# facebookresearch/iSDF

Hardware: AMD Instinct MI355X
Metric: train-steps/sec: device-synchronised Trainer.step() on 27k-point ray batches, timed as metrics.start_timing / end_timing bracket it (SURVEY 8d); whole job.  SDF L1 vs GT: sdf_l1_vs_gt (higher is better)
Workload: dtype f16 MFMA operands (compensated forward: hi+lo operands past the cat layer), f32 accumulate; second-order sweeps and dW operands fp16; 1 GPU; replicaCAD.json defaults: 5 keyframes x 200 rays x 27 samples = 27000 points per rank-step, 680x1200 synthetic room depth, 6x256 Softplus MLP + 255-wide icosahedron PE (460033 params), eik+normal loss, bounds=ray, AdamW; stream=680x1200, scaling_mode=weak: every rank draws the full 5 x 200 rays, parallelism=single GPU

## Files before the change

### isdf_amd/csrc/capi.hip

```cpp
#include <cstdio>
#include "isdf_common.h"
#include "chain_params.h"
#include "launchers.h"

using namespace isdf;

namespace isdf { thread_local int g_isdf_last_hip_error = 0; }

extern "C" {

int isdf_abi_version(void) { return ISDF_ABI_VERSION; }

static thread_local int g_isdf_last_collective_error = 0;

const char* isdf_error_string(int code) {
  switch (code) {
    case ISDF_OK: return "ok";
    case ISDF_EINVAL: return "invalid argument";
    case ISDF_EUNSUPPORTED: return "unsupported configuration (the tile kernels take hidden_feature_size <= 512 (zero-padded to 256 / 512), n_freqs = n_embed_funcs+1 in 1..12, any hidden_layers_block up to 7; bounds_method ray|pc)";
    case ISDF_EWORKSPACE: return "workspace too small";
    case ISDF_EHIP: {
      static thread_local char buf[160];
      snprintf(buf, sizeof(buf), "HIP runtime error: %s", g_isdf_last_hip_error ? hipGetErrorString((hipError_t)g_isdf_last_hip_error) : "(no launch status recorded)");
      return buf;
// ... 70 lines not shown
  if (!scan_ws || scan_ws_bytes < sample_scan_bytes((int64_t)a->n_frames * a->n_rays)) return ISDF_EWORKSPACE;
  return launch_sample_rays(*a, *o, scan_ws, (hipStream_t)stream);
}

int isdf_sdf_eval(const isdf_net_cfg* net, const float* params, const void* shadow, const float* pts,
                  int64_t n_points, const float* noise, float* sdf, float* sdf_grad, void* workspace,
                  int64_t workspace_bytes, void* stream) {
  isdf_clear_stale_hip_error();
  NetLayout l; int rc = make_layout(net, &l);
  if (rc) return rc;
  if (!layout_supported(l)) return ISDF_EUNSUPPORTED;
  if (!params || !shadow || !pts || !sdf || n_points < 0) return ISDF_EINVAL;
  if (n_points == 0) return ISDF_OK;
  ChainParams p = {};
  p.lay = l; p.params = params; p.shadow = (const uint16_t*)shadow; p.pts = pts; p.noise = noise;
  p.n_points_host = n_points; p.S = 1; p.sdf = sdf; p.sdf_grad = sdf_grad;
  const int mode = sdf_grad ? 1 : 0;
  WorkspaceLayout w; make_workspace(l, n_points, 0, false, &w);
  if (mode == 1) {
    if (!workspace || workspace_bytes < w.totalBytes) return ISDF_EWORKSPACE;
    p.spill = (uint16_t*)((char*)workspace + w.offSpill); p.sp = w.sp;
  }
  chain_debug_from_env(p.dbg, workspace && workspace_bytes >= 4096 ? (char*)workspace + workspace_bytes - 4096 : nullptr);
  return launch_chain(p, mode, w.nTiles, (hipStream_t)stream);
}

static bool optim_args_ok(const isdf_optim_args* opt, int32_t n_frames) {
  if (!opt || !opt->params || !opt->exp_avg || !opt->exp_avg_sq || !opt->shadow || opt->step < 1) return false;
  if ((opt->loss_approx == nullptr) != (opt->frame_avg == nullptr)) return false;
  if (opt->frame_avg_inline_n != 0 && (opt->frame_avg_inline_n != n_frames || opt->frame_avg_inline_n > ISDF_MAX_INLINE_FRAMES))
    return false;
// ... 32 lines not shown
  const int64_t maxPts = (int64_t)a->max_rays * a->S;
  if (maxPts > 0x7fffffff) return ISDF_EINVAL;
  if (a->extra_floats < 0 || a->extra_floats > 1016 || (a->extra_floats > 0 && (a->extra_slot < 0 || a->extra_slot >= a->extra_floats)))
    return ISDF_EINVAL;
  WorkspaceLayout w; make_workspace(l, maxPts, a->max_rays, true, &w);
  if (workspace_bytes < w.totalBytes) return ISDF_EWORKSPACE;
  hipStream_t st = (hipStream_t)stream;
  char* ws = (char*)workspace;
  float* wgLoss = (float*)(ws + w.offWgLoss);
  float* dwPart = (float*)(ws + w.offDwPart);
  float* vecPart = (float*)(ws + w.offVecPart);
  float* totLoss = (float*)(ws + w.offTotLoss);

  ChainParams p = {};
  p.lay = l; p.loss = *loss; p.params = params; p.shadow = (const uint16_t*)shadow;
  p.pts = a->pc; p.noise = a->noise; p.n_valid = a->n_valid; p.S = a->S;
  p.noise_std = a->noise_std; p.noise_seed = a->noise_seed; p.noise_off = a->noise_offset;
  p.z_vals = a->z_vals; p.depth = a->depth_sample; p.dirsC = a->dirs_C_sample; p.dirsW = a->dirs_W_sample;
  p.normals = a->norm_sample; p.pc_bounds = a->pc_bounds; p.pc_grad_vec = a->pc_grad_vec;
  p.sdf = o->sdf; p.sdf_grad = o->sdf_grad; p.tot_loss_mat = o->tot_loss_mat;
  p.tot_ws = totLoss; p.wg_loss = wgLoss; p.vec_part = vecPart; p.vecStride = w.vecStride;
  p.spill = (uint16_t*)(ws + w.offSpill); p.sp = w.sp;
  p.pe_aux = (float*)(ws + w.offPeAux);
  chain_debug_from_env(p.dbg, ws + w.totalBytes - 4096);
  hipEvent_t* ev = (hipEvent_t*)o->prof_events;
  if (ev && hipEventRecord(ev[0], st) != hipSuccess) return ISDF_EHIP;
  rc = launch_chain(p, 2, w.nTiles, st);
  if (rc) return rc;
  if (ev && hipEventRecord(ev[1], st) != hipSuccess) return ISDF_EHIP;

  DwParams d = {};
  d.lay = l; d.sp = w.sp; d.spill = p.spill; d.pe_aux = p.pe_aux; d.n_valid = a->n_valid; d.S = a->S; d.dwPart = dwPart;
  rc = launch_dw(d, st);
  if (rc) return rc;
  if (ev && hipEventRecord(ev[2], st) != hipSuccess) return ISDF_EHIP;
  const ReduceLayout r = reduce_layout(l, a->n_frames);
  TailParams t = {};
  t.lay = l; t.dwPart = dwPart; t.vecPart = vecPart; t.vecStride = w.vecStride; t.grad = o->reduce_buf;
  FinalizeArgs& f = t.fin;
  f.wg_loss = wgLoss; f.maxTiles = w.nTiles; f.n_valid = a->n_valid; f.S = a->S; f.tot_ws = totLoss;
  f.ib = a->indices_b; f.ih = a->indices_h; f.iw = a->indices_w; f.n_frames = a->n_frames; f.H = a->H; f.W = a->W;
  f.loss_sums = o->reduce_buf + r.lossSums; f.block_loss = o->reduce_buf + r.blockLoss; f.block_cnt = o->reduce_buf + r.blockCnt;
  f.mailbox = o->host_mailbox; f.extra = o->reduce_buf + r.extra;
  f.n_extra = a->extra_floats; f.extra_slot = a->extra_slot; f.extra_value = a->extra_value;
  if (opt) {
    const AdamwHyper hyper = tail_optim(t, *opt);
    rc = launch_step_tail(0, t, &hyper, 0, st);
// ... 301 lines not shown
```

### isdf_amd/csrc/chain.hip

```cpp
#include <atomic>
#include "chain_dev.h"
#include "launchers.h"

namespace isdf {

constexpr bool oper_f16(int oper) { return oper >= 1; }
constexpr bool oper_x2(int oper) { return oper >= 2; }
constexpr bool oper_x2_all(int oper) { return oper == 3; }

template <int HD, int EP, bool LO_REGIONS = false>
struct Tile {
  static constexpr int BM = TILE_PTS;
  static constexpr int NW = CHAIN_NW;
  static constexpr int CKF = CHAIN_CHUNK_FRAGS;
  static constexpr int FB = HD / (NW * 32);
  static constexpr int PB = BM / 32;
  static constexpr int R2 = (EP > HD ? EP : HD);
  static constexpr int XK = (HD + R2) * (LO_REGIONS ? 2 : 1);
  static constexpr int ROWB = XK * 2;
  static constexpr int XBYTES = BM * ROWB;
  static constexpr int OFF_XS = XBYTES;
  static constexpr bool WIDE_E = EP > HD;
  static constexpr int NPART = WIDE_E ? (NW * 64) / 32 : (NW * 64) / BM;
  static constexpr int OFF_PART = OFF_XS + BM * 16;
// ... 4 lines not shown
};

template <int FBN, int CKF> struct WChunk { uint4 v[CKF / FBN][FBN]; };
struct WRef { int soff; int rb; };

template <int FBN, int CKF>
__device__ __forceinline__ void load_w(WChunk<FBN, CKF>& wq, rsrc_t rw, WRef r, int lane16, int chunk) {
  constexpr int CK = CKF / FBN;
#pragma unroll
  for (int s = 0; s < CK; ++s)
#pragma unroll
    for (int fb = 0; fb < FBN; ++fb)
      wq.v[s][fb] = bload16<0>(rw, lane16 + (s & 3) * 1024, r.soff + fb * r.rb + chunk * CK * 1024 + (s >> 2) * 4096);
}

template <bool F16, int KSTEPS, int FBN, int PBN, int ROWB, int CKF, bool ZERO = false, bool TWO = false, typename Hook>
__device__ __forceinline__ void gemm(f32x16 (&acc)[FBN][PBN], WChunk<FBN, CKF>& wq, rsrc_t rw, WRef wr, const char* xl,
                                     int colByteBase, int lane, Hook&& postHook, int colByteBase2 = 0) {
  constexpr int CK = CKF / FBN;
  static_assert(KSTEPS % CK == 0, "K must be a multiple of the chunk");
  static_assert((ROWB & 255) == 0, "row base must leave the swizzle bits (4-7) clear");
  constexpr int NCH = KSTEPS / CK;
  typedef typename Op<F16>::v8 v8;
  const int j = lane & 31, hi = lane >> 5;
  const int xlane = j * ROWB + ((hi * 16) ^ ((j & 15) << 4));
  const int lane16 = lane * 16;
  load_w(wq, rw, wr, lane16, 0);
  auto chunk = [&](int ch, auto refill, auto zero) {
    const int k0 = ch * CK;
    int xch = (xlane ^ ((k0 & 7) * 32)) + (k0 >> 3) * 256 + colByteBase;
    asm volatile("" : "+v"(xch));
    constexpr int NB = TWO ? 2 * PBN : PBN;
    auto readb = [&](int s, v8 (&b)[NB]) {
#pragma unroll
      for (int pb = 0; pb < PBN; ++pb)
        b[pb] = __builtin_bit_cast(v8, *(const uint4*)(xl + ((xch ^ (s * 32)) + pb * 32 * ROWB)));
      if constexpr (TWO) {
#pragma unroll
        for (int pb = 0; pb < PBN; ++pb)
          b[PBN + pb] = __builtin_bit_cast(v8, *(const uint4*)(xl + ((xch ^ (s * 32)) + pb * 32 * ROWB + (colByteBase2 - colByteBase))));
      }
    };
// ... 57 lines not shown
  float* gbs = (float*)(smem + T::OFF_GB);
  float* red = (float*)(smem + T::OFF_RED);

  const NetLayout& L = p.lay;
  const int tid = threadIdx.x;
  const int w = __builtin_amdgcn_readfirstlane(tid >> 6);
  static_assert(FB <= 2, "the LDS write addressing below assumes one or two feature blocks per wave");
  int lane, j, hi, lane16, xw;
  auto refresh = [&] {
    int t = tid;
    asm volatile("" : "+v"(t));
    lane = t & 63; j = lane & 31; hi = lane >> 5; lane16 = lane * 16;
    xw = j * ROWB + 8 * hi + (((j & 15) << 4) ^ (((w * FB) & 3) * 64)) + ((w * FB) >> 2) * 256;
  };
  refresh();
  const int64_t P = p.n_valid ? (int64_t)(*p.n_valid) * p.S : p.n_points_host;
  const int64_t n0 = (int64_t)blockIdx.x * BM;
  if (n0 >= P) return;
  const int nf = L.n_freqs;
  const float so = L.scale_output;
  ChainStamps TS(p.dbg, p.n_cu);
  TS();
  if (SP8) __builtin_amdgcn_s_setreg(1 | (23 << 6), 1);
  const bool genOdd = ((int)blockIdx.x / p.n_cu) & 1;
  auto PRIO = [&](int phase) {
    if (genOdd) { if (phase == 1 || phase == 2) __builtin_amdgcn_s_setprio(1); else __builtin_amdgcn_s_setprio(0); }
  };
  PRIO(0);
  TS.wall(0);

  const int64_t setFwdA = L.setFwdA, setFwdB = L.setFwdB, setBwdA = L.setBwdA, setBwdB = L.setBwdB, setFwdLo = L.setFwdLo;
  uint16_t* spillTile = p.spill + TS.spill_tile() * p.sp.tileStride;
  const rsrc_t rsW = make_rsrc(p.shadow, 0x7fffffffu);
  const rsrc_t rsS = make_rsrc(spillTile, (uint32_t)(p.sp.tileStride * 2));
  const i32x4 srdS = make_srd(spillTile, (uint32_t)(p.sp.tileStride * 2));
  auto sbase = [&](int64_t tensorOff) { return (int)(tensorOff * 2) + w * (FB * PB * 2) * 1024; };
  constexpr auto cidx = [](int fb, int pb, int qp) { return (fb * PB + pb) * 2 + qp; };
  float* vecTile = MODE == 2 ? p.vec_part + (int64_t)blockIdx.x * p.vecStride : nullptr;
  const rsrc_t rsV = make_rsrc(vecTile, MODE == 2 ? (uint32_t)p.vecStride * 4u : 0u);
  (void)setFwdB; (void)setBwdB; (void)setFwdLo; (void)rsS; (void)rsV; (void)srdS;
  auto ubase = [&](int fb, int qp) { return w * (FB * 32) + fb * 32 + 16 * qp; };
  auto ld_params8 = [&](int vecBase, int ub, float (&o)[8]) {
    const rsrc_t rv = make_rsrc(p.params + vecBase, (uint32_t)L.H * 4u);
    const u32x4 a = __builtin_amdgcn_raw_buffer_load_b128(rv, 16 * hi, ub * 4, 0);
    const u32x4 b = __builtin_amdgcn_raw_buffer_load_b128(rv, 16 * hi + 32, ub * 4, 0);
#pragma unroll
    for (int e = 0; e < 4; ++e) { o[e] = __uint_as_float(a[e]); o[4 + e] = __uint_as_float(b[e]); }
  };
  auto vec_store8 = [&](float (&v)[8], int elemUniform) {
#pragma unroll
    for (int e = 0; e < 8; ++e) v[e] = half_wave_sum(v[e]);
    const bool b0 = j & 1, b1 = j & 2, b2 = j & 4;
    const float t0 = b0 ? v[1] : v[0], t1 = b0 ? v[3] : v[2], t2 = b0 ? v[5] : v[4], t3 = b0 ? v[7] : v[6];
    const float u0 = b1 ? t1 : t0, u1 = b1 ? t3 : t2;
    const float r = b2 ? u1 : u0;
    if (j < 8) __builtin_amdgcn_raw_buffer_store_b32(__float_as_uint(r), rsV, 16 * hi + 4 * (j & 3) + 32 * (j >> 2), elemUniform * 4, 0);
  };

  if constexpr (!WIDE_E && BM == 64) {
    const int ln = tid & 63;
    const int64_t n = n0 + ln;
    float x0 = 0.f, x1 = 0.f, x2 = 0.f;
    if (n < P) { x0 = p.pts[n * 3]; x1 = p.pts[n * 3 + 1]; x2 = p.pts[n * 3 + 2]; }
    const float y0 = (L.T[0] * x0 + L.T[1] * x1 + L.T[2] * x2 + L.T[3]) * L.scale_input;
    const float y1 = (L.T[4] * x0 + L.T[5] * x1 + L.T[6] * x2 + L.T[7]) * L.scale_input;
    const float y2 = (L.T[8] * x0 + L.T[9] * x1 + L.T[10] * x2 + L.T[11]) * L.scale_input;
    typedef typename Op<F16>::e opT;
    const int sw = (ln & 15) << 4;
    char* row = X + ln * ROWB;
    auto put = [&](int feat, float v) {
      *(opT*)(row + (((HD + feat) * 2) ^ sw)) = (opT)v;
      if (X2ALL) *(opT*)(row + (((LO + HD + feat) * 2) ^ sw)) = (opT)(v - (float)(opT)v);
    };
    if (w == T::NW - 1) {
      xs[ln * 4] = y0; xs[ln * 4 + 1] = y1; xs[ln * 4 + 2] = y2;
      put(0, y0); put(1, y1); put(2, y2);
      for (int f = L.E; f < EP; ++f) put(f, 0.f);
    }
    for (int d = w; d < N_DIRS; d += T::NW) {
      const float proj = y0 * kDirs[0][d] + y1 * kDirs[1][d] + y2 * kDirs[2][d];
      float fr = 1.f;
      for (int f = 0; f < nf; ++f) {
        const float xb = proj * fr;
        put(3 + d * nf + f, __sinf(xb));
        put(3 + N_DIRS * nf + d * nf + f, __sinf(xb + kHalfPi));
        fr *= 2.f;
      }
    }
  } else
  {
    const int pt = (tid % (BM / T::NW)) + (BM / T::NW) * (tid / 64), prt = (tid % 64) / (BM / T::NW);
    constexpr int NPART = (T::NW * 64) / BM;
    const int64_t n = n0 + pt;
    float x0 = 0.f, x1 = 0.f, x2 = 0.f;
    if (n < P) { x0 = p.pts[n * 3]; x1 = p.pts[n * 3 + 1]; x2 = p.pts[n * 3 + 2]; }
    float y0 = (L.T[0] * x0 + L.T[1] * x1 + L.T[2] * x2 + L.T[3]) * L.scale_input;
    float y1 = (L.T[4] * x0 + L.T[5] * x1 + L.T[6] * x2 + L.T[7]) * L.scale_input;
    float y2 = (L.T[8] * x0 + L.T[9] * x1 + L.T[10] * x2 + L.T[11]) * L.scale_input;
    typedef typename Op<F16>::e opT;
    char* row = X + pt * ROWB;
    auto put = [&](int feat, float v) {
      *(opT*)(row + swz(pt, (HD + feat) * 2)) = (opT)v;
      if (X2ALL) *(opT*)(row + swz(pt, (LO + HD + feat) * 2)) = (opT)(v - (float)(opT)v);
    };
    if (prt == 0) {
      xs[pt * 4] = y0; xs[pt * 4 + 1] = y1; xs[pt * 4 + 2] = y2;
      put(0, y0); put(1, y1); put(2, y2);
      for (int f = L.E; f < EP; ++f) put(f, 0.f);
    }
    for (int d = prt; d < N_DIRS; d += NPART) {
      const float proj = y0 * kDirs[0][d] + y1 * kDirs[1][d] + y2 * kDirs[2][d];
      float fr = 1.f;
      for (int f = 0; f < nf; ++f) {
        const float xb = proj * fr;
        put(3 + d * nf + f, __sinf(xb));
        put(3 + N_DIRS * nf + d * nf + f, __sinf(xb + kHalfPi));
        fr *= 2.f;
      }
    }
  }
  lds_barrier();
  refresh();

  f32x16 acc[FB][PB];
  const int rbW = w * FB;
  auto wptr = [&](int64_t set, int64_t matOff, int kp) {
    return WRef{(int)((set + matOff) * 2) + rbW * (kp / 16) * 1024, (kp / 16) * 1024};
  };
  auto fwdW = [&](int64_t set, int li) {
    return wptr(set, L.fwdMat[li], li == 0 ? EP : (li == L.cat ? HD + EP : HD));
  };
  WChunk<FB, T::CKF> wq;
  WChunk<FB, T::CKF / 2> wq2;
  auto for_blocks2 = [&](auto&& fn, auto&& tail) {
#pragma unroll
    for (int fb = 0; fb < FB; ++fb)
#pragma unroll
      for (int qp = 0; qp < 2; ++qp) {
#pragma unroll
        for (int pb = 0; pb < PB; ++pb) fn(fb, pb, qp, pb * 32 + j);
        tail(fb, qp);
      }
  };
  auto for_blocks = [&](auto&& fn) { for_blocks2(fn, [](int, int) {}); };
  struct Pre { uint4 v[FB][2][PB]; };
  auto prefetch = [&](int64_t tensorOff, Pre& pr) {
    const int sb = sbase(tensorOff);
#pragma unroll
// ... 92 lines not shown
#pragma unroll
  for (int pb = 0; pb < PB; ++pb) rawp[pb] = 0.f;

  auto put_x_hilo = [&](int fb, int pb, int qp, const float (&v)[8]) {
    f16x4 ha, hb;
    float r[8];
#pragma unroll
    for (int e = 0; e < 4; ++e) { ha[e] = (_Float16)v[e]; hb[e] = (_Float16)v[4 + e]; }
#pragma unroll
    for (int e = 0; e < 4; ++e) { r[e] = v[e] - (float)ha[e]; r[4 + e] = v[4 + e] - (float)hb[e]; }
    const int lb = (xw ^ (64 * fb + 32 * qp)) + pb * 32 * ROWB;
    *(uint2*)(X + lb) = __builtin_bit_cast(uint2, ha);
    *(uint2*)(X + (lb ^ 16)) = __builtin_bit_cast(uint2, hb);
    put_x(true, fb, pb, qp, r, LO);
  };
  for (int li = 0; li < L.L; ++li) {
    refresh();
    const bool comp = X2 && (X2ALL || li >= L.cat);
    if (li == 0) {
      if (X2ALL) {
        gemm<F16, EP / 16, FB, PB, ROWB, T::CKF / 2, true, true>(acc, wq2, rsW, fwdW(setFwdA, li), X, HD * 2, lane, [] {}, (LO + HD) * 2);
        gemm<F16, EP / 16, FB, PB, ROWB, T::CKF>(acc, wq, rsW, fwdW(setFwdLo, li), X, HD * 2, lane, [] {});
      } else {
        gemm<F16, EP / 16, FB, PB, ROWB, T::CKF, true>(acc, wq, rsW, fwdW(setFwdA, li), X, HD * 2, lane, [] {});
      }
    } else if (li == L.cat) {
      if (X2ALL) {
        gemm<F16, (HD + EP) / 16, FB, PB, ROWB, T::CKF / 2, true, true>(acc, wq2, rsW, fwdW(setFwdA, li), X, 0, lane, [] {}, LO * 2);
        gemm<F16, (HD + EP) / 16, FB, PB, ROWB, T::CKF>(acc, wq, rsW, fwdW(setFwdLo, li), X, 0, lane, [] {});
      } else {
        gemm<F16, (HD + EP) / 16, FB, PB, ROWB, T::CKF, true>(acc, wq, rsW, fwdW(setFwdA, li), X, 0, lane, [] {});
      }
      if (!X2ALL && comp) {
        WRef wl = fwdW(setFwdLo, li);
        wl.soff += (HD / 16) * 1024;
        gemm<F16, EP / 16, FB, PB, ROWB, T::CKF>(acc, wq, rsW, wl, X, HD * 2, lane, [] {});
      }
    } else {
      if (comp) {
        gemm<F16, HD / 16, FB, PB, ROWB, T::CKF / 2, true, true>(acc, wq2, rsW, fwdW(setFwdA, li), X, 0, lane, [] {}, LO * 2);
        gemm<F16, HD / 16, FB, PB, ROWB, T::CKF>(acc, wq, rsW, fwdW(setFwdLo, li), X, 0, lane, [] {});
      } else {
        gemm<F16, HD / 16, FB, PB, ROWB, T::CKF, true>(acc, wq, rsW, fwdW(setFwdA, li), X, 0, lane, [] {});
      }
    }
    TS();
    lds_barrier();
    TS();
    refresh();
    const bool last = li == L.L - 1;
    if (!last) {
      float bv[8];
      for_blocks([&](int fb, int pb, int qp, int row) {
        if (pb == 0) ld_params8(L.offB[li], ubase(fb, qp), bv);
        float a[8];
#pragma unroll
        for (int e = 0; e < 8; ++e) a[e] = softplus_f(acc[fb][pb][8 * qp + e] + bv[e]);
        if (MODE >= 1) store_tile8(p.sp.A[li + 1], fb, pb, qp, a);
        if (X2 && (X2ALL || li + 1 > L.cat)) put_x_hilo(fb, pb, qp, a);
        else put_x(F16, fb, pb, qp, a, 0);
      });
    } else {
      float bv[8], wv[8];
      for_blocks([&](int fb, int pb, int qp, int row) {
        if (pb == 0) {
          ld_params8(L.offB[li], ubase(fb, qp), bv);
          ld_params8(L.offWout, ubase(fb, qp), wv);
        }
        float a[8], pl[8];
#pragma unroll
        for (int e = 0; e < 8; ++e) {
          float s1;
          a[e] = softplus_s1(acc[fb][pb][8 * qp + e] + bv[e], s1);
          pl[e] = so * wv[e] * s1;
        }
        f32x2 r2 = {0.f, 0.f};
#pragma unroll
        for (int e = 0; e < 8; e += 2) r2 += f32x2{wv[e], wv[e + 1]} * f32x2{a[e], a[e + 1]};
        rawp[pb] += r2[0] + r2[1];
        if (MODE >= 1) {
          store_tile8(p.sp.A[li + 1], fb, pb, qp, a);
          put_x(F16, fb, pb, qp, pl, 0);
          if (MODE == 2) store_tile8(p.sp.P[li], fb, pb, qp, pl);
        }
      });
    }
    if (last) {
#pragma unroll
      for (int pb = 0; pb < PB; ++pb) {
        const float v = rawp[pb] + __shfl_xor(rawp[pb], 32, 64);
        if (hi == 0) part[(w * BM + pb * 32 + j) * 4] = v;
      }
    }
    TS();
    lds_barrier();
    TS();
  }
  float my_sdf = 0.f;
  if (tid < BM) {
    float r = p.params[L.offBout];
#pragma unroll
    for (int k = 0; k < T::NW; ++k) r += part[(k * BM + tid) * 4];
    const int64_t n = n0 + tid;
    if (p.noise) { if (n < P) r += p.noise[n]; }
    else if (p.noise_std != 0.f) {
      const uint4 u = philox4x32_10(make_uint4((uint32_t)n, (uint32_t)(n >> 32), (uint32_t)p.noise_off, (uint32_t)(p.noise_off >> 32)),
                                    make_uint2((uint32_t)p.noise_seed, (uint32_t)(p.noise_seed >> 32) ^ 0x5eedu));
      const float u1 = fmaxf(u01(u.x), 1e-7f), u2 = u01(u.y);
      r += p.noise_std * sqrtf(-2.f * __logf(u1)) * __cosf(6.2831853f * u2);
    }
    my_sdf = r * so;
    if (p.sdf && n < P) p.sdf[n] = my_sdf;
  }
  if (MODE == 0) return;

// ... 530 lines not shown
```

### isdf_amd/csrc/chain_params.h

```cpp
#pragma once
#include "isdf_common.h"
#include "chain_debug.h"

namespace isdf {

struct ChainParams {
  NetLayout lay;
  isdf_loss_cfg loss;
  const float* params;
  const uint16_t* shadow;
  const float* pts;
  const float* noise;
  float noise_std; uint64_t noise_seed, noise_off;
  const int32_t* n_valid;
  int64_t n_points_host;
  int32_t S;
  const float* z_vals; const float* depth; const float* dirsC; const float* dirsW; const float* normals;
  const float* pc_bounds; const float* pc_grad_vec;
  float* sdf; float* sdf_grad; float* tot_loss_mat;
  float* tot_ws;
  float* wg_loss;
  float* vec_part;
  int32_t vecStride;
  uint16_t* spill; SpillLayout sp;
  float* pe_aux;
  int32_t n_cu;
  ChainDebug dbg;
};

struct DwParams {
  NetLayout lay;
  SpillLayout sp;
  const uint16_t* spill;
  const float* pe_aux;
  const int32_t* n_valid; int64_t n_points_host; int32_t S;
  float* dwPart;
};

struct AdamwHyper { float lr, b1, b2, eps, wd; int step; };
struct AdamwCoef { float lr, b1, b2, eps, wd, bc1, bc2_sqrt; };
struct FinalizeArgs {
  const float* wg_loss; int64_t maxTiles; const int32_t* n_valid; int S; const float* tot_ws;
  const int64_t *ib, *ih, *iw; int n_frames, H, W;
  float *loss_sums, *block_loss, *block_cnt;
  float *la_out, *fa_out; const int32_t* fa_index;
  int fa_inline_n; int32_t fa_inline[8];
  float* mailbox; float* extra; int n_extra, extra_slot; float extra_value;
};
static_assert(ISDF_MAX_INLINE_FRAMES == 8, "FinalizeArgs::fa_inline holds isdf_optim_args.frame_avg_index_inline");
struct TailParams {
// ... 13 lines not shown
```

### isdf_amd/csrc/dw.hip

```cpp
#include "isdf_common.h"
#include "launchers.h"
#include "chain_params.h"
#include "chain_dev.h"

namespace isdf {


template <int HD> struct DwTile {
  static constexpr int BM = DW_PTS;
  static constexpr int NT = 256;
  static constexpr int ROWB = DW_BLK * 2 + 64;
  static constexpr int TEN = BM * ROWB;
  static constexpr int AUXB = BM * 32;
  static constexpr int DIRTAB = 4 * TEN + 2 * AUXB;
  static constexpr int DUMMY = DIRTAB + 512;
  static constexpr int LDS_BYTES = DUMMY + ROWB;
  static constexpr int CH = (BM * DW_BLK * 2) / (NT * 16);
};

__device__ __forceinline__ int frag16_piece(int c, int half, int sl, int& pt, int& f0) {
  constexpr int PB = TILE_PTS / 32, HB = DW_PTS / 32;
  const int lane = c & 63; int r = c >> 6;
  const int qp = r & 1; r >>= 1;
  const int pbh = r % HB; const int blk = r / HB;
  pt = pbh * 32 + (lane & 31);
  f0 = blk * 32 + 16 * qp + 4 * (lane >> 5);
  return ((((sl * 8 + blk) * PB + half * HB + pbh) * 2 + qp) * 64 + lane);
}

template <int HD, bool F16, int SP8>
__global__ __launch_bounds__(256, 1) void dw_kernel(const DwParams p) {
  typedef DwTile<HD> T;
  constexpr int BM = T::BM, ROWB = T::ROWB, CH = T::CH, NT = T::NT;
  static_assert(TILE_PTS == DW_PTS, "pe_aux staging below assumes one dW stage pair per chain tile");
  static_assert(CH == 8 && BM / 16 == 4, "one 16-bit chunk rides behind each of the eight half-steps (an e4m3 chunk behind every other)");
  extern __shared__ __attribute__((aligned(16))) char smem[];
  const NetLayout& L = p.lay;
  const int tid = threadIdx.x, lane = tid & 63, w = tid >> 6;
  const int wo = w >> 1, wi = w & 1;
  int unit = 0, split = blockIdx.x;
  for (int n; split >= (n = dw_unit_splits(L, unit)); ++unit) split -= n;
  const int DW_SPLITK = dw_unit_splits(L, unit);
  const DwUnit du = dw_unit(L, unit);
  const int li = du.li;
  const bool fromEmb = dw_unit_from_emb(L, du);
  const int slBfull = (li == L.cat && fromEmb) ? du.ib - HD / DW_BLK : du.ib;
  const int slB = slBfull % (HD / DW_BLK);
  const int slA = du.ob;
  if (fromEmb && slBfull * DW_BLK >= L.E) return;

  const int64_t P = p.n_valid ? (int64_t)(*p.n_valid) * p.S : p.n_points_host;
  const int nTiles = (int)((P + TILE_PTS - 1) / TILE_PTS);

  const int64_t offZ = p.sp.ZB[li], offP = p.sp.P[li];
  const int64_t offI = fromEmb ? 0 : p.sp.A[li];
  const int64_t offG = fromEmb ? 0 : p.sp.GB[li];
  constexpr int CH8 = CH / 2;

  f32x16 acc[4][4];
#pragma unroll
  for (int a = 0; a < 4; ++a)
#pragma unroll
    for (int b = 0; b < 4; ++b)
#pragma unroll
      for (int r = 0; r < 16; ++r) acc[a][b][r] = 0.f;

  const int nStages = split < nTiles ? 2 * ((nTiles - split + DW_SPLITK - 1) / DW_SPLITK) : 0;
  const bool peAligned = fromEmb && slBfull == 0 && L.E <= DW_BLK && L.n_freqs == 6;

  const int s16 = lane & 15, cg = (lane >> 4) & 1, hi = lane >> 5;
  const int trRow = 8 * hi + (s16 >> 2);
  const int trColB = (16 * cg + 4 * (s16 & 3)) * 2;
  const int trX = ((trRow >> 1) & 7) << 3;
  const int trOffA = trRow * ROWB + (trColB ^ trX), trOffB = (trRow + 4) * ROWB + (trColB ^ trX ^ 16);
  const int trOffA_in = fromEmb ? trRow * ROWB + trColB : trOffA, trOffB_in = fromEmb ? (trRow + 4) * ROWB + trColB : trOffB;
  int pt16, f16;
  const int vo16 = frag16_piece(tid, 0, 0, pt16, f16) * 16, vo8 = tid * 16;
  const int wr16A = pt16 * ROWB + ((f16 * 2) ^ (((pt16 >> 1) & 7) << 3)), wr16B = wr16A ^ 16;
  const int f8 = (w >> 1) * 32 + 16 * (w & 1) + 4 * (lane >> 5);
  const int wr8A = (lane & 31) * ROWB + ((f8 * 2) ^ ((((lane & 31) >> 1) & 7) << 3)), wr8B = wr8A ^ 16;
  typedef bf16x4 __attribute__((address_space(3))) * lds4;
  auto trload = [&](const char* base, int ptBase, int colElem, int offA, int offB) -> bf16x8 {
// ... 46 lines not shown
    loadB(sb, 2, b0); loadA(sb, 2, 0, a0);      mfmas(I1{}, a1, b1); between(I1{}, I1{});
    loadA(sb, 2, 1, a1);                        mfmas(I0{}, a0, b0); between(I2{}, I0{});
    loadB(sb, 3, b1); loadA(sb, 3, 0, a0);      mfmas(I1{}, a1, b0); between(I2{}, I1{});
    loadA(sb, 3, 1, a1);                        mfmas(I0{}, a0, b1); between(I3{}, I0{});
                                                mfmas(I1{}, a1, b1); between(I3{}, I1{});
  };

  auto run = [&](auto pe_tag, auto p8_tag, auto nft_tag, auto slice_tag) {
    constexpr bool PE = decltype(pe_tag)::value;
    constexpr int NFT = decltype(nft_tag)::value, SLT = decltype(slice_tag)::value;
    constexpr bool ALIGNED = NFT == 6;
    constexpr bool p8 = decltype(p8_tag)::value, g8 = SP8 & 1;
    constexpr int CHA1 = p8 ? CH8 : CH, CHB1 = g8 ? CH8 : CH;
    uint4 regA0[CH], regB0[CH], regA1[CHA1], regB1[CHB1];
    float sG1[2] = {1.f, 1.f};
    const int tileBytes = (int)p.sp.tileStride * 2;
    auto tile_rsrc = [&](int64_t off, int t) { return make_rsrc(p.spill + off + (int64_t)t * p.sp.tileStride, (uint32_t)tileBytes); };
    auto issue0 = [&](int st, auto cTag) {
      constexpr int c = decltype(cTag)::value;
      const int t = split + (st >> 1) * DW_SPLITK;
      regA0[c] = bload16<kAuxDwLoad>(tile_rsrc(offZ, t), vo16, slA * 32768 + c * 4096);
      if constexpr (!PE) regB0[c] = bload16<kAuxDwLoad>(tile_rsrc(offI, t), vo16, slB * 32768 + c * 4096);
    };
    auto issue1 = [&](int st, auto ksTag, auto hTag) {
      constexpr int ks = decltype(ksTag)::value, h = decltype(hTag)::value, c = 2 * ks + h;
      const int t = split + (st >> 1) * DW_SPLITK;
      if constexpr (p8) { if constexpr (h == 0) regA1[ks] = bload16<kAuxDwLoad>(tile_rsrc(offP, t), vo8, slA * 16384 + ks * 4096); }
      else regA1[c] = bload16<kAuxDwLoad>(tile_rsrc(offP, t), vo16, slA * 32768 + c * 4096);
      if constexpr (!PE) {
        if constexpr (g8) {
          if constexpr (h == 1) regB1[ks] = bload16<kAuxDwLoad>(tile_rsrc(offG, t), vo8, slB * 16384 + ks * 4096);
          if constexpr (ks == 3 && h == 1) {
            const rsrc_t rx = make_rsrc(p.pe_aux + (int64_t)t * BM * 8, BM * 32);
            sG1[0] = __builtin_bit_cast(float, __builtin_amdgcn_raw_buffer_load_b32(rx, (tid & 31) * 32 + 28, 0, 0));
            sG1[1] = __builtin_bit_cast(float, __builtin_amdgcn_raw_buffer_load_b32(rx, (tid & 31) * 32 + 28, 32 * 32, 0));
          }
        } else {
          regB1[c] = bload16<kAuxDwLoad>(tile_rsrc(offG, t), vo16, slB * 32768 + c * 4096);
        }
      }
    };
    auto cvt2 = [](uint32_t w8, float scale, auto hiTag) -> uint32_t {
      if constexpr (F16) return __builtin_bit_cast(uint32_t, __builtin_amdgcn_cvt_scalef32_pk_f16_fp8((int)w8, scale, decltype(hiTag)::value));
      else return __builtin_bit_cast(uint32_t, __builtin_amdgcn_cvt_scalef32_pk_bf16_fp8((int)w8, scale, decltype(hiTag)::value));
    };
    constexpr float kInv2Pi = 0.15915494309189535f, k2Pi = 6.283185307179586f;
    constexpr int NR = (BM * N_DIRS + BM + NT - 1) / NT;
    float4 auxr = make_float4(0.f, 0.f, 0.f, 0.f);
    if constexpr (PE) {
      if (tid < N_DIRS)
        *(float4*)(smem + T::DIRTAB + tid * 16) = make_float4(kDirs[0][tid] * kInv2Pi, kDirs[1][tid] * kInv2Pi, kDirs[2][tid] * kInv2Pi, 0.f);
    }
    auto load_aux = [&](int k) {
      k = min(k, nStages / 2 - 1);
      const uint4 v = bload16<0>(make_rsrc(p.pe_aux + (int64_t)(split + k * DW_SPLITK) * BM * 8, BM * 32), (tid & 127) * 16, 0);
      auxr = make_float4(__uint_as_float(v.x), __uint_as_float(v.y), __uint_as_float(v.z), __uint_as_float(v.w));
    };
    auto store_aux = [&](int k) {
      *(float4*)(smem + 4 * T::TEN + (k & 1) * T::AUXB + (tid & 127) * 16) = auxr;
    };
    auto put16 = [&](char* tile, const auto& r, auto cTag) {
      constexpr int c = decltype(cTag)::value;
      *(uint2*)(tile + wr16A + c * 64) = make_uint2(r[c].x, r[c].y);
      *(uint2*)(tile + wr16B + c * 64) = make_uint2(r[c].z, r[c].w);
    };
    auto put8 = [&](char* tile, const auto& r, float s0, float s1, auto cTag) {
      constexpr int c = decltype(cTag)::value;
      const uint4 a = r[c];
      *(uint2*)(tile + wr8A + c * 128) = make_uint2(cvt2(a.x, s0, std::false_type{}), cvt2(a.x, s0, std::true_type{}));
      *(uint2*)(tile + wr8B + c * 128) = make_uint2(cvt2(a.y, s0, std::false_type{}), cvt2(a.y, s0, std::true_type{}));
      *(uint2*)(tile + wr8A + 32 * ROWB + c * 128) = make_uint2(cvt2(a.z, s1, std::false_type{}), cvt2(a.z, s1, std::true_type{}));
      *(uint2*)(tile + wr8B + 32 * ROWB + c * 128) = make_uint2(cvt2(a.w, s1, std::false_type{}), cvt2(a.w, s1, std::true_type{}));
// ... 108 lines not shown
    };
    auto issue = [&](int st, auto oddTag, auto ksTag, auto hTag) {
      constexpr int ks = decltype(ksTag)::value, h = decltype(hTag)::value;
      constexpr bool ODD = decltype(oddTag)::value;
      st = min(st, nStages - (ODD ? 1 : 2));
      if constexpr (ODD) issue1(st, ksTag, hTag);
      else issue0(st, std::integral_constant<int, 2 * ks + h>{});
    };
    auto each_slice = [&](auto&& fn) {
      typedef std::integral_constant<int, 0> I0; typedef std::integral_constant<int, 1> I1;
      fn(I0{}, I0{}); fn(I0{}, I1{}); fn(I1{}, I0{}); fn(I1{}, I1{});
      fn(std::integral_constant<int, 2>{}, I0{}); fn(std::integral_constant<int, 2>{}, I1{});
      fn(std::integral_constant<int, 3>{}, I0{}); fn(std::integral_constant<int, 3>{}, I1{});
    };

    if constexpr (PE) {
      load_aux(0); store_aux(0); load_aux(1);
      if constexpr (NFT != 0 && !ALIGNED && SLT == 1) {
        constexpr int c0 = 3 + 2 * N_DIRS * NFT - DW_BLK, npad = DW_BLK - c0;
        typedef typename Op<F16>::e eT0;
        for (int i = tid; i < BM * npad; i += NT) {
          const int r = i / npad, c = c0 + i - r * npad;
          *(eT0*)(smem + T::TEN + r * ROWB + c * 2) = (eT0)0.f;
          *(eT0*)(smem + 3 * T::TEN + r * ROWB + c * 2) = (eT0)0.f;
        }
      }
    }
    each_slice([&](auto k, auto h) { issue(0, std::false_type{}, k, h); });
    each_slice([&](auto k, auto h) { issue(1, std::true_type{}, k, h); });
    if constexpr (PE) __syncthreads();
    if constexpr (PE) fill_fetch(0, std::false_type{}, std::integral_constant<int, 0>{});
    each_slice([&](auto k, auto h) { commit(0, std::false_type{}, k, h); issue(2, std::false_type{}, k, h); });
    __syncthreads();

    typedef std::integral_constant<int, PE ? 12 : 4> NV;
    typedef std::integral_constant<int, PE ? 2 : 1> NW;
    for (int st = 0; st < nStages; st += 2) {
      compute(0, NV{}, NW{}, [&] { if constexpr (PE) fill_fetch(st + 1, std::true_type{}, std::integral_constant<int, 0>{}); },
              [&](auto ks, auto h) {
        commit(st + 1, std::true_type{}, ks, h);
        issue(st + 3, std::true_type{}, ks, h);
        if constexpr (PE && decltype(ks)::value == 3 && decltype(h)::value == 1) { store_aux((st >> 1) + 1); load_aux((st >> 1) + 2); }
      });
      __syncthreads();
      compute(1, NV{}, NW{}, [&] { if constexpr (PE) fill_fetch(st + 2, std::false_type{}, std::integral_constant<int, 0>{}); },
              [&](auto ks, auto h) {
        commit(st + 2, std::false_type{}, ks, h);
        issue(st + 4, std::false_type{}, ks, h);
      });
      __syncthreads();
    }
  };
  typedef std::integral_constant<bool, (SP8 & 2) != 0> P8T;
  typedef std::integral_constant<int, 0> I0_; typedef std::integral_constant<int, 1> I1_;
  const bool straightRef = SP8 == 0 && fromEmb && L.EP == 2 * DW_BLK && (L.n_freqs == 9 || L.n_freqs == 11);
  if (nStages == 0) {}
  else if (fromEmb && peAligned) run(std::true_type{}, P8T{}, std::integral_constant<int, 6>{}, I0_{});
  else if (straightRef) {
    if constexpr (SP8 == 0) {
      if (L.n_freqs == 9) { if (slBfull == 0) run(std::true_type{}, P8T{}, std::integral_constant<int, 9>{}, I0_{}); else run(std::true_type{}, P8T{}, std::integral_constant<int, 9>{}, I1_{}); }
      else { if (slBfull == 0) run(std::true_type{}, P8T{}, std::integral_constant<int, 11>{}, I0_{}); else run(std::true_type{}, P8T{}, std::integral_constant<int, 11>{}, I1_{}); }
    }
  }
  else if (fromEmb) run(std::true_type{}, P8T{}, std::integral_constant<int, 0>{}, I0_{});
  else if ((SP8 & 2) && li == L.L - 1) run(std::false_type{}, std::false_type{}, std::integral_constant<int, 0>{}, I0_{});
  else run(std::false_type{}, P8T{}, std::integral_constant<int, 0>{}, I0_{});

  slab_t* slab = (slab_t*)p.dwPart + ((int64_t)dw_slab_base(L, unit) + split) * DW_BLK * DW_BLK;
#pragma unroll
  for (int ob = 0; ob < 4; ++ob)
#pragma unroll
    for (int ib = 0; ib < 4; ++ib)
// ... 34 lines not shown
```

Before: 3875 train-steps/s.

## Hoist n_valid-dependent loads ahead of the count read in chain and dW kernels

Both the chain and dW kernels now issue their first global loads before they read the device-side n_valid count: points, first-layer weights, biases and the output bias in the chain kernel, and the first spill/aux stages in the dW kernel. These loads are bounds-limited by buffer capacity (new pts_capacity and cap_tiles fields) rather than by the valid count, so the count fetch's latency overlaps with useful loads instead of serialising in front of them. The forward layers also prefetch the next layer's bias and output weights inside the GEMM post-hook, replacing per-block parameter loads in the epilogue. The cost is extra registers for the prefetched parameters and wasted speculative loads for tiles that end up past the valid count.

```diff
diff --git a/isdf_amd/csrc/capi.hip b/isdf_amd/csrc/capi.hip
--- a/isdf_amd/csrc/capi.hip
+++ b/isdf_amd/csrc/capi.hip
@@ -108,7 +108,7 @@
   if (n_points == 0) return ISDF_OK;
   ChainParams p = {};
   p.lay = l; p.params = params; p.shadow = (const uint16_t*)shadow; p.pts = pts; p.noise = noise;
-  p.n_points_host = n_points; p.S = 1; p.sdf = sdf; p.sdf_grad = sdf_grad;
+  p.n_points_host = n_points; p.pts_capacity = n_points; p.S = 1; p.sdf = sdf; p.sdf_grad = sdf_grad;
   const int mode = sdf_grad ? 1 : 0;
   WorkspaceLayout w; make_workspace(l, n_points, 0, false, &w);
   if (mode == 1) {
@@ -171,7 +171,7 @@
 
   ChainParams p = {};
   p.lay = l; p.loss = *loss; p.params = params; p.shadow = (const uint16_t*)shadow;
-  p.pts = a->pc; p.noise = a->noise; p.n_valid = a->n_valid; p.S = a->S;
+  p.pts = a->pc; p.pts_capacity = maxPts; p.noise = a->noise; p.n_valid = a->n_valid; p.S = a->S;
   p.noise_std = a->noise_std; p.noise_seed = a->noise_seed; p.noise_off = a->noise_offset;
   p.z_vals = a->z_vals; p.depth = a->depth_sample; p.dirsC = a->dirs_C_sample; p.dirsW = a->dirs_W_sample;
   p.normals = a->norm_sample; p.pc_bounds = a->pc_bounds; p.pc_grad_vec = a->pc_grad_vec;
@@ -187,7 +187,8 @@
   if (ev && hipEventRecord(ev[1], st) != hipSuccess) return ISDF_EHIP;
 
   DwParams d = {};
-  d.lay = l; d.sp = w.sp; d.spill = p.spill; d.pe_aux = p.pe_aux; d.n_valid = a->n_valid; d.S = a->S; d.dwPart = dwPart;
+  d.lay = l; d.sp = w.sp; d.spill = p.spill; d.pe_aux = p.pe_aux; d.n_valid = a->n_valid; d.S = a->S; d.cap_tiles = (int32_t)w.nTiles;
+  d.dwPart = dwPart;
   rc = launch_dw(d, st);
   if (rc) return rc;
   if (ev && hipEventRecord(ev[2], st) != hipSuccess) return ISDF_EHIP;
diff --git a/isdf_amd/csrc/chain.hip b/isdf_amd/csrc/chain.hip
--- a/isdf_amd/csrc/chain.hip
+++ b/isdf_amd/csrc/chain.hip
@@ -42,7 +42,7 @@
       wq.v[s][fb] = bload16<0>(rw, lane16 + (s & 3) * 1024, r.soff + fb * r.rb + chunk * CK * 1024 + (s >> 2) * 4096);
 }
 
-template <bool F16, int KSTEPS, int FBN, int PBN, int ROWB, int CKF, bool ZERO = false, bool TWO = false, typename Hook>
+template <bool F16, int KSTEPS, int FBN, int PBN, int ROWB, int CKF, bool ZERO = false, bool TWO = false, bool PRE = false, typename Hook>
 __device__ __forceinline__ void gemm(f32x16 (&acc)[FBN][PBN], WChunk<FBN, CKF>& wq, rsrc_t rw, WRef wr, const char* xl,
                                      int colByteBase, int lane, Hook&& postHook, int colByteBase2 = 0) {
   constexpr int CK = CKF / FBN;
@@ -53,7 +53,7 @@
   const int j = lane & 31, hi = lane >> 5;
   const int xlane = j * ROWB + ((hi * 16) ^ ((j & 15) << 4));
   const int lane16 = lane * 16;
-  load_w(wq, rw, wr, lane16, 0);
+  if constexpr (!PRE) load_w(wq, rw, wr, lane16, 0);
   auto chunk = [&](int ch, auto refill, auto zero) {
     const int k0 = ch * CK;
     int xch = (xlane ^ ((k0 & 7) * 32)) + (k0 >> 3) * 256 + colByteBase;
@@ -141,9 +141,44 @@
     xw = j * ROWB + 8 * hi + (((j & 15) << 4) ^ (((w * FB) & 3) * 64)) + ((w * FB) >> 2) * 256;
   };
   refresh();
-  const int64_t P = p.n_valid ? (int64_t)(*p.n_valid) * p.S : p.n_points_host;
   const int64_t n0 = (int64_t)blockIdx.x * BM;
+  const rsrc_t rsW = make_rsrc(p.shadow, 0x7fffffffu);
+  auto ubase = [&](int fb, int qp) { return w * (FB * 32) + fb * 32 + 16 * qp; };
+  auto ld_params8 = [&](int vecBase, int ub, int hq, float (&o)[8]) {
+    const rsrc_t rv = make_rsrc(p.params + vecBase, (uint32_t)L.H * 4u);
+    const u32x4 a = __builtin_amdgcn_raw_buffer_load_b128(rv, 16 * hq, ub * 4, 0);
+    const u32x4 b = __builtin_amdgcn_raw_buffer_load_b128(rv, 16 * hq + 32, ub * 4, 0);
+#pragma unroll
+    for (int e = 0; e < 4; ++e) { o[e] = __uint_as_float(a[e]); o[4 + e] = __uint_as_float(b[e]); }
+  };
+  const int rbW = w * FB;
+  auto wptr = [&](int64_t set, int64_t matOff, int kp) {
+    return WRef{(int)((set + matOff) * 2) + rbW * (kp / 16) * 1024, (kp / 16) * 1024};
+  };
+  auto fwdW = [&](int64_t set, int li) {
+    return wptr(set, L.fwdMat[li], li == 0 ? EP : (li == L.cat ? HD + EP : HD));
+  };
+  WChunk<FB, T::CKF> wq;
+  WChunk<FB, T::CKF / 2> wq2;
+  int nvRaw = (int)__builtin_amdgcn_raw_buffer_load_b32(make_rsrc(p.n_valid, p.n_valid ? 4u : 0u), 0, 0, 0);
+  const int prow = (!WIDE_E && BM == 64) ? (tid & 63) : (tid % (BM / T::NW)) + (BM / T::NW) * (tid / 64);
+  const int64_t capLeft = p.pts_capacity - n0;
+  const rsrc_t rsP = make_rsrc(p.pts + n0 * 3, (uint32_t)(capLeft < 0 ? 0 : (capLeft < BM ? capLeft : BM)) * 12u);
+  float px0 = __uint_as_float(__builtin_amdgcn_raw_buffer_load_b32(rsP, prow * 12, 0, 0));
+  float px1 = __uint_as_float(__builtin_amdgcn_raw_buffer_load_b32(rsP, prow * 12 + 4, 0, 0));
+  float px2 = __uint_as_float(__builtin_amdgcn_raw_buffer_load_b32(rsP, prow * 12 + 8, 0, 0));
+  if constexpr (X2ALL) load_w(wq2, rsW, fwdW(L.setFwdA, 0), lane16, 0);
+  else load_w(wq, rsW, fwdW(L.setFwdA, 0), lane16, 0);
+  float bvq[FB][2][8];
+#pragma unroll
+  for (int fb = 0; fb < FB; ++fb)
+#pragma unroll
+    for (int qp = 0; qp < 2; ++qp) ld_params8(L.offB[0], ubase(fb, qp), hi, bvq[fb][qp]);
+  const float b_out = __uint_as_float(__builtin_amdgcn_raw_buffer_load_b32(make_rsrc(p.params + L.offBout, 4u), 0, 0, 0));
+  asm volatile("" : "+v"(nvRaw) : : "memory");
+  const int64_t P = p.n_valid ? (int64_t)__builtin_amdgcn_readfirstlane(nvRaw) * p.S : p.n_points_host;
   if (n0 >= P) return;
+  if (n0 + prow >= P) { px0 = 0.f; px1 = 0.f; px2 = 0.f; }
   const int nf = L.n_freqs;
   const float so = L.scale_output;
   ChainStamps TS(p.dbg, p.n_cu);
@@ -158,7 +193,6 @@
 
   const int64_t setFwdA = L.setFwdA, setFwdB = L.setFwdB, setBwdA = L.setBwdA, setBwdB = L.setBwdB, setFwdLo = L.setFwdLo;
   uint16_t* spillTile = p.spill + TS.spill_tile() * p.sp.tileStride;
-  const rsrc_t rsW = make_rsrc(p.shadow, 0x7fffffffu);
   const rsrc_t rsS = make_rsrc(spillTile, (uint32_t)(p.sp.tileStride * 2));
   const i32x4 srdS = make_srd(spillTile, (uint32_t)(p.sp.tileStride * 2));
   auto sbase = [&](int64_t tensorOff) { return (int)(tensorOff * 2) + w * (FB * PB * 2) * 1024; };
@@ -166,14 +200,6 @@
   float* vecTile = MODE == 2 ? p.vec_part + (int64_t)blockIdx.x * p.vecStride : nullptr;
   const rsrc_t rsV = make_rsrc(vecTile, MODE == 2 ? (uint32_t)p.vecStride * 4u : 0u);
   (void)setFwdB; (void)setBwdB; (void)setFwdLo; (void)rsS; (void)rsV; (void)srdS;
-  auto ubase = [&](int fb, int qp) { return w * (FB * 32) + fb * 32 + 16 * qp; };
-  auto ld_params8 = [&](int vecBase, int ub, float (&o)[8]) {
-    const rsrc_t rv = make_rsrc(p.params + vecBase, (uint32_t)L.H * 4u);
-    const u32x4 a = __builtin_amdgcn_raw_buffer_load_b128(rv, 16 * hi, ub * 4, 0);
-    const u32x4 b = __builtin_amdgcn_raw_buffer_load_b128(rv, 16 * hi + 32, ub * 4, 0);
-#pragma unroll
-    for (int e = 0; e < 4; ++e) { o[e] = __uint_as_float(a[e]); o[4 + e] = __uint_as_float(b[e]); }
-  };
   auto vec_store8 = [&](float (&v)[8], int elemUniform) {
 #pragma unroll
     for (int e = 0; e < 8; ++e) v[e] = half_wave_sum(v[e]);
@@ -186,9 +212,7 @@
 
   if constexpr (!WIDE_E && BM == 64) {
     const int ln = tid & 63;
-    const int64_t n = n0 + ln;
-    float x0 = 0.f, x1 = 0.f, x2 = 0.f;
-    if (n < P) { x0 = p.pts[n * 3]; x1 = p.pts[n * 3 + 1]; x2 = p.pts[n * 3 + 2]; }
+    const float x0 = px0, x1 = px1, x2 = px2;
     const float y0 = (L.T[0] * x0 + L.T[1] * x1 + L.T[2] * x2 + L.T[3]) * L.scale_input;
     const float y1 = (L.T[4] * x0 + L.T[5] * x1 + L.T[6] * x2 + L.T[7]) * L.scale_input;
     const float y2 = (L.T[8] * x0 + L.T[9] * x1 + L.T[10] * x2 + L.T[11]) * L.scale_input;
@@ -218,9 +242,7 @@
   {
     const int pt = (tid % (BM / T::NW)) + (BM / T::NW) * (tid / 64), prt = (tid % 64) / (BM / T::NW);
     constexpr int NPART = (T::NW * 64) / BM;
-    const int64_t n = n0 + pt;
-    float x0 = 0.f, x1 = 0.f, x2 = 0.f;
-    if (n < P) { x0 = p.pts[n * 3]; x1 = p.pts[n * 3 + 1]; x2 = p.pts[n * 3 + 2]; }
+    const float x0 = px0, x1 = px1, x2 = px2;
     float y0 = (L.T[0] * x0 + L.T[1] * x1 + L.T[2] * x2 + L.T[3]) * L.scale_input;
     float y1 = (L.T[4] * x0 + L.T[5] * x1 + L.T[6] * x2 + L.T[7]) * L.scale_input;
     float y2 = (L.T[8] * x0 + L.T[9] * x1 + L.T[10] * x2 + L.T[11]) * L.scale_input;
@@ -250,15 +272,6 @@
   refresh();
 
   f32x16 acc[FB][PB];
-  const int rbW = w * FB;
-  auto wptr = [&](int64_t set, int64_t matOff, int kp) {
-    return WRef{(int)((set + matOff) * 2) + rbW * (kp / 16) * 1024, (kp / 16) * 1024};
-  };
-  auto fwdW = [&](int64_t set, int li) {
-    return wptr(set, L.fwdMat[li], li == 0 ? EP : (li == L.cat ? HD + EP : HD));
-  };
-  WChunk<FB, T::CKF> wq;
-  WChunk<FB, T::CKF / 2> wq2;
   auto for_blocks2 = [&](auto&& fn, auto&& tail) {
 #pragma unroll
     for (int fb = 0; fb < FB; ++fb)
@@ -381,34 +394,51 @@
     *(uint2*)(X + (lb ^ 16)) = __builtin_bit_cast(uint2, hb);
     put_x(true, fb, pb, qp, r, LO);
   };
-  for (int li = 0; li < L.L; ++li) {
+  auto fwd_layer = [&](int li, auto firstTag) {
+    constexpr bool FIRST = decltype(firstTag)::value;
     refresh();
     const bool comp = X2 && (X2ALL || li >= L.cat);
-    if (li == 0) {
+    float wvq[FB][2][8];
+    auto top_params = [&] {
+      if (li != L.L - 1) return;
+#pragma unroll
+      for (int fb = 0; fb < FB; ++fb)
+#pragma unroll
+        for (int qp = 0; qp < 2; ++qp) ld_params8(L.offWout, ubase(fb, qp), lane >> 5, wvq[fb][qp]);
+    };
+    auto fwd_params = [&] {
+#pragma unroll
+      for (int fb = 0; fb < FB; ++fb)
+#pragma unroll
+        for (int qp = 0; qp < 2; ++qp) ld_params8(L.offB[li], ubase(fb, qp), lane >> 5, bvq[fb][qp]);
+      top_params();
+    };
+    if constexpr (FIRST) {
       if (X2ALL) {
-        gemm<F16, EP / 16, FB, PB, ROWB, T::CKF / 2, true, true>(acc, wq2, rsW, fwdW(setFwdA, li), X, HD * 2, lane, [] {}, (LO + HD) * 2);
-        gemm<F16, EP / 16, FB, PB, ROWB, T::CKF>(acc, wq, rsW, fwdW(setFwdLo, li), X, HD * 2, lane, [] {});
+        gemm<F16, EP / 16, FB, PB, ROWB, T::CKF / 2, true, true, true>(acc, wq2, rsW, fwdW(setFwdA, li), X, HD * 2, lane, [] {}, (LO + HD) * 2);
+        gemm<F16, EP / 16, FB, PB, ROWB, T::CKF>(acc, wq, rsW, fwdW(setFwdLo, li), X, HD * 2, lane, top_params);
       } else {
-        gemm<F16, EP / 16, FB, PB, ROWB, T::CKF, true>(acc, wq, rsW, fwdW(setFwdA, li), X, HD * 2, lane, [] {});
+        gemm<F16, EP / 16, FB, PB, ROWB, T::CKF, true, false, true>(acc, wq, rsW, fwdW(setFwdA, li), X, HD * 2, lane, top_params);
       }
     } else if (li == L.cat) {
+      constexpr bool LO3 = X2 && !X2ALL;
       if (X2ALL) {
         gemm<F16, (HD + EP) / 16, FB, PB, ROWB, T::CKF / 2, true, true>(acc, wq2, rsW, fwdW(setFwdA, li), X, 0, lane, [] {}, LO * 2);
-        gemm<F16, (HD + EP) / 16, FB, PB, ROWB, T::CKF>(acc, wq, rsW, fwdW(setFwdLo, li), X, 0, lane, [] {});
+        gemm<F16, (HD + EP) / 16, FB, PB, ROWB, T::CKF>(acc, wq, rsW, fwdW(setFwdLo, li), X, 0, lane, fwd_params);
       } else {
-        gemm<F16, (HD + EP) / 16, FB, PB, ROWB, T::CKF, true>(acc, wq, rsW, fwdW(setFwdA, li), X, 0, lane, [] {});
-      }
-      if (!X2ALL && comp) {
+        gemm<F16, (HD + EP) / 16, FB, PB, ROWB, T::CKF, true>(acc, wq, rsW, fwdW(setFwdA, li), X, 0, lane, [&] { if constexpr (!LO3) fwd_params(); });
+      }
+      if constexpr (LO3) {
         WRef wl = fwdW(setFwdLo, li);
         wl.soff += (HD / 16) * 1024;
-        gemm<F16, EP / 16, FB, PB, ROWB, T::CKF>(acc, wq, rsW, wl, X, HD * 2, lane, [] {});
+        gemm<F16, EP / 16, FB, PB, ROWB, T::CKF>(acc, wq, rsW, wl, X, HD * 2, lane, fwd_params);
       }
     } else {
       if (comp) {
         gemm<F16, HD / 16, FB, PB, ROWB, T::CKF / 2, true, true>(acc, wq2, rsW, fwdW(setFwdA, li), X, 0, lane, [] {}, LO * 2);
-        gemm<F16, HD / 16, FB, PB, ROWB, T::CKF>(acc, wq, rsW, fwdW(setFwdLo, li), X, 0, lane, [] {});
+        gemm<F16, HD / 16, FB, PB, ROWB, T::CKF>(acc, wq, rsW, fwdW(setFwdLo, li), X, 0, lane, fwd_params);
       } else {
-        gemm<F16, HD / 16, FB, PB, ROWB, T::CKF, true>(acc, wq, rsW, fwdW(setFwdA, li), X, 0, lane, [] {});
+        gemm<F16, HD / 16, FB, PB, ROWB, T::CKF, true>(acc, wq, rsW, fwdW(setFwdA, li), X, 0, lane, fwd_params);
       }
     }
     TS();
@@ -417,9 +447,8 @@
     refresh();
     const bool last = li == L.L - 1;
     if (!last) {
-      float bv[8];
       for_blocks([&](int fb, int pb, int qp, int row) {
-        if (pb == 0) ld_params8(L.offB[li], ubase(fb, qp), bv);
+        const float (&bv)[8] = bvq[fb][qp];
         float a[8];
 #pragma unroll
         for (int e = 0; e < 8; ++e) a[e] = softplus_f(acc[fb][pb][8 * qp + e] + bv[e]);
@@ -428,12 +457,8 @@
         else put_x(F16, fb, pb, qp, a, 0);
       });
     } else {
-      float bv[8], wv[8];
       for_blocks([&](int fb, int pb, int qp, int row) {
-        if (pb == 0) {
-          ld_params8(L.offB[li], ubase(fb, qp), bv);
-          ld_params8(L.offWout, ubase(fb, qp), wv);
-        }
+        const float (&bv)[8] = bvq[fb][qp], (&wv)[8] = wvq[fb][qp];
         float a[8], pl[8];
 #pragma unroll
         for (int e = 0; e < 8; ++e) {
@@ -462,10 +487,12 @@
     TS();
     lds_barrier();
     TS();
-  }
+  };
+  fwd_layer(0, std::true_type{});
+  for (int li = 1; li < L.L; ++li) fwd_layer(li, std::false_type{});
   float my_sdf = 0.f;
   if (tid < BM) {
-    float r = p.params[L.offBout];
+    float r = b_out;
 #pragma unroll
     for (int k = 0; k < T::NW; ++k) r += part[(k * BM + tid) * 4];
     const int64_t n = n0 + tid;
diff --git a/isdf_amd/csrc/chain_params.h b/isdf_amd/csrc/chain_params.h
--- a/isdf_amd/csrc/chain_params.h
+++ b/isdf_amd/csrc/chain_params.h
@@ -14,6 +14,7 @@
   float noise_std; uint64_t noise_seed, noise_off;
   const int32_t* n_valid;
   int64_t n_points_host;
+  int64_t pts_capacity;
   int32_t S;
   const float* z_vals; const float* depth; const float* dirsC; const float* dirsW; const float* normals;
   const float* pc_bounds; const float* pc_grad_vec;
@@ -34,6 +35,7 @@
   const uint16_t* spill;
   const float* pe_aux;
   const int32_t* n_valid; int64_t n_points_host; int32_t S;
+  int32_t cap_tiles;
   float* dwPart;
 };
 
diff --git a/isdf_amd/csrc/dw.hip b/isdf_amd/csrc/dw.hip
--- a/isdf_amd/csrc/dw.hip
+++ b/isdf_amd/csrc/dw.hip
@@ -36,6 +36,8 @@
   static_assert(CH == 8 && BM / 16 == 4, "one 16-bit chunk rides behind each of the eight half-steps (an e4m3 chunk behind every other)");
   extern __shared__ __attribute__((aligned(16))) char smem[];
   const NetLayout& L = p.lay;
+  const int32_t nvRaw = (int32_t)__builtin_amdgcn_raw_buffer_load_b32(make_rsrc(p.n_valid, p.n_valid ? 4u : 0u), 0, 0, 0);
+  asm volatile("" ::: "memory");
   const int tid = threadIdx.x, lane = tid & 63, w = tid >> 6;
   const int wo = w >> 1, wi = w & 1;
   int unit = 0, split = blockIdx.x;
@@ -49,8 +51,8 @@
   const int slA = du.ob;
   if (fromEmb && slBfull * DW_BLK >= L.E) return;
 
-  const int64_t P = p.n_valid ? (int64_t)(*p.n_valid) * p.S : p.n_points_host;
-  const int nTiles = (int)((P + TILE_PTS - 1) / TILE_PTS);
+  const bool tileInBuf = split < p.cap_tiles;
+  const uint32_t tileBytes = tileInBuf ? (uint32_t)p.sp.tileStride * 2u : 0u, auxBytes = tileInBuf ? (uint32_t)(BM * 32) : 0u;
 
   const int64_t offZ = p.sp.ZB[li], offP = p.sp.P[li];
   const int64_t offI = fromEmb ? 0 : p.sp.A[li];
@@ -65,7 +67,6 @@
 #pragma unroll
       for (int r = 0; r < 16; ++r) acc[a][b][r] = 0.f;
 
-  const int nStages = split < nTiles ? 2 * ((nTiles - split + DW_SPLITK - 1) / DW_SPLITK) : 0;
   const bool peAligned = fromEmb && slBfull == 0 && L.E <= DW_BLK && L.n_freqs == 6;
 
   const int s16 = lane & 15, cg = (lane >> 4) & 1, hi = lane >> 5;
@@ -142,8 +143,8 @@
     constexpr int CHA1 = p8 ? CH8 : CH, CHB1 = g8 ? CH8 : CH;
     uint4 regA0[CH], regB0[CH], regA1[CHA1], regB1[CHB1];
     float sG1[2] = {1.f, 1.f};
-    const int tileBytes = (int)p.sp.tileStride * 2;
-    auto tile_rsrc = [&](int64_t off, int t) { return make_rsrc(p.spill + off + (int64_t)t * p.sp.tileStride, (uint32_t)tileBytes); };
+    int nStages = 0;
+    auto tile_rsrc = [&](int64_t off, int t) { return make_rsrc(p.spill + off + (int64_t)t * p.sp.tileStride, tileBytes); };
     auto issue0 = [&](int st, auto cTag) {
       constexpr int c = decltype(cTag)::value;
       const int t = split + (st >> 1) * DW_SPLITK;
@@ -159,7 +160,7 @@
         if constexpr (g8) {
           if constexpr (h == 1) regB1[ks] = bload16<kAuxDwLoad>(tile_rsrc(offG, t), vo8, slB * 16384 + ks * 4096);
           if constexpr (ks == 3 && h == 1) {
-            const rsrc_t rx = make_rsrc(p.pe_aux + (int64_t)t * BM * 8, BM * 32);
+            const rsrc_t rx = make_rsrc(p.pe_aux + (int64_t)t * BM * 8, auxBytes);
             sG1[0] = __builtin_bit_cast(float, __builtin_amdgcn_raw_buffer_load_b32(rx, (tid & 31) * 32 + 28, 0, 0));
             sG1[1] = __builtin_bit_cast(float, __builtin_amdgcn_raw_buffer_load_b32(rx, (tid & 31) * 32 + 28, 32 * 32, 0));
           }
@@ -179,11 +180,11 @@
       if (tid < N_DIRS)
         *(float4*)(smem + T::DIRTAB + tid * 16) = make_float4(kDirs[0][tid] * kInv2Pi, kDirs[1][tid] * kInv2Pi, kDirs[2][tid] * kInv2Pi, 0.f);
     }
-    auto load_aux = [&](int k) {
-      k = min(k, nStages / 2 - 1);
-      const uint4 v = bload16<0>(make_rsrc(p.pe_aux + (int64_t)(split + k * DW_SPLITK) * BM * 8, BM * 32), (tid & 127) * 16, 0);
+    auto load_aux_at = [&](int k) {
+      const uint4 v = bload16<0>(make_rsrc(p.pe_aux + (int64_t)(split + k * DW_SPLITK) * BM * 8, auxBytes), (tid & 127) * 16, 0);
       auxr = make_float4(__uint_as_float(v.x), __uint_as_float(v.y), __uint_as_float(v.z), __uint_as_float(v.w));
     };
+    auto load_aux = [&](int k) { load_aux_at(min(k, nStages / 2 - 1)); };
     auto store_aux = [&](int k) {
       *(float4*)(smem + 4 * T::TEN + (k & 1) * T::AUXB + (tid & 127) * 16) = auxr;
     };
@@ -322,8 +323,20 @@
       fn(std::integral_constant<int, 3>{}, I0{}); fn(std::integral_constant<int, 3>{}, I1{});
     };
 
+    if constexpr (PE) load_aux_at(0);
+    each_slice([&](auto k, auto h) { issue0(0, std::integral_constant<int, 2 * decltype(k)::value + decltype(h)::value>{}); });
+    each_slice([&](auto k, auto h) { issue1(1, k, h); });
+    {
+      int nv = nvRaw;
+      asm volatile("" : "+v"(nv) : : "memory");
+      nv = __builtin_amdgcn_readfirstlane(nv);
+      const int64_t P = p.n_valid ? (int64_t)nv * p.S : p.n_points_host;
+      const int nTiles = (int)((P + TILE_PTS - 1) / TILE_PTS);
+      nStages = split < nTiles ? 2 * ((nTiles - split + DW_SPLITK - 1) / DW_SPLITK) : 0;
+    }
+    if (nStages == 0) return;
     if constexpr (PE) {
-      load_aux(0); store_aux(0); load_aux(1);
+      store_aux(0); load_aux(1);
       if constexpr (NFT != 0 && !ALIGNED && SLT == 1) {
         constexpr int c0 = 3 + 2 * N_DIRS * NFT - DW_BLK, npad = DW_BLK - c0;
         typedef typename Op<F16>::e eT0;
@@ -334,8 +347,6 @@
         }
       }
     }
-    each_slice([&](auto k, auto h) { issue(0, std::false_type{}, k, h); });
-    each_slice([&](auto k, auto h) { issue(1, std::true_type{}, k, h); });
     if constexpr (PE) __syncthreads();
     if constexpr (PE) fill_fetch(0, std::false_type{}, std::integral_constant<int, 0>{});
     each_slice([&](auto k, auto h) { commit(0, std::false_type{}, k, h); issue(2, std::false_type{}, k, h); });
@@ -362,8 +373,7 @@
   typedef std::integral_constant<bool, (SP8 & 2) != 0> P8T;
   typedef std::integral_constant<int, 0> I0_; typedef std::integral_constant<int, 1> I1_;
   const bool straightRef = SP8 == 0 && fromEmb && L.EP == 2 * DW_BLK && (L.n_freqs == 9 || L.n_freqs == 11);
-  if (nStages == 0) {}
-  else if (fromEmb && peAligned) run(std::true_type{}, P8T{}, std::integral_constant<int, 6>{}, I0_{});
+  if (fromEmb && peAligned) run(std::true_type{}, P8T{}, std::integral_constant<int, 6>{}, I0_{});
   else if (straightRef) {
     if constexpr (SP8 == 0) {
       if (L.n_freqs == 9) { if (slBfull == 0) run(std::true_type{}, P8T{}, std::integral_constant<int, 9>{}, I0_{}); else run(std::true_type{}, P8T{}, std::integral_constant<int, 9>{}, I1_{}); }
```

New measurement: 3923 train-steps/s (median of 6 runs). 1.2% higher.
